# dscripka/openWakeWord

Hardware: NVIDIA H100
Metric: 80ms audio-frames/sec (concurrent streams) (higher is better)
Workload: dtype f16 operands / f32 accumulate (mel, BN, LayerNorm, sigmoid in f32; heads' first layer as fp16 hi/lo split = f32-grade)

## Files before the change

### openwakeword_b200/csrc/cnn_tc_inc.cu

```cuda
#include "oww_internal.h"
#include "tc_common.cuh"
#include "mel_device.cuh"
#include <cmath>
#include <cstring>
#include <type_traits>

namespace {

constexpr int kIncEpiWarps = 16;
constexpr int kIncThreads = kIncEpiWarps * 32;
constexpr int kIncMaxG = 7;
constexpr int kMelNF = 2;

__device__ __forceinline__ __half2 u32_as_half2(uint32_t v) {
    return __halves2half2(__ushort_as_half((unsigned short)(v & 0xFFFFu)), __ushort_as_half((unsigned short)(v >> 16)));
}

struct IncArgs {
    IncPlan plan;
    const float* mel; const int* mel_count; int64_t mel_stride; int mel_mask; int back;
    const float* w0; const float* s0; const float* b0;
    const uint8_t* wblob;
    const uint4* tails_in; uint4* tails_out;
    float* emb;
    int B;
    const int* live_chunks; int live_min;
    long long* dbg_clock;
// ... 73 lines not shown
        mbar_expect_tx(hfull(slot), bytes);
        bulk_g2s(smem_u32(smem + a.hring_off + slot * a.hslot_bytes), src, bytes, hfull(slot));
        ++hchunk_p;
        return true;
    };

    const int et = threadIdx.x;
    uint32_t epar[2] = {0, 0};
    uint32_t epi_tails_par = 0, mma_tails_par = 0;
    uint32_t hf_par = 0; int hchunk_e = 0;
    for (int grp = blockIdx.x; grp < P.n_groups; grp += gridDim.x) {
        const uint4* tin = a.tails_in + (int64_t)grp * P.tail_units;
        uint4* tout = a.tails_out + (int64_t)grp * P.tail_units;
        int* s_cnt = reinterpret_cast<int*>(smem + 512);
        int* s_live = s_cnt + 16;
        float* s_mel = reinterpret_cast<float*>(smem + P.scratch_off + 6144);
        if (a.dbg_clock && blockIdx.x == 0 && grp == 0 && et == 0) a.dbg_clock[101] = clock64();
        named_bar_sync(2, kIncEpiWarps * 32);
        if (et < G) {
            const int b = grp * G + et;
            s_live[et] = b < a.B && (!a.live_chunks || a.live_chunks[b] >= a.live_min);
        }
        named_bar_sync(2, kIncEpiWarps * 32);
        if (fused) {
            uint8_t* sc = smem + P.scratch_off;
            float2* s_tw = reinterpret_cast<float2*>(sc);
            float* s_win = reinterpret_cast<float*>(sc + 4096);
            uint8_t* s_work = smem + 2048 + warp * (kMelNF * kMelFrameScratch);
            float* s_floor = s_mel + G * 256;
            int seen_v = 1;
            for (int i = et; i < 512; i += kIncEpiWarps * 32) { s_tw[i] = a.mel_twiddle[i]; s_win[i] = a.mel_window[i]; }
            if (et < G) {
                const int b = grp * G + et;
                s_cnt[et] = s_live[et] ? a.mel_count_rw[b] : 0;
                s_cnt[8 + et] = s_live[et] ? a.feat_count[b] : 0;
                seen_v = s_live[et] ? a.seen[b] : 1;
                s_live[8 + et] = s_live[et] && seen_v == 0;
            }
            named_bar_sync(2, kIncEpiWarps * 32);
            const int my_start = a.mel_start[lane], my_len = a.mel_len[lane];
            const float* my_w = a.mel_w + lane * OWW_MEL_MAXSUPPORT;
            for (int fi = warp * kMelNF; fi < G * 8; fi += kIncEpiWarps * kMelNF) {
                const int16_t* tl[kMelNF]; const int16_t* bd[kMelNF]; int fr[kMelNF]; float db[kMelNF];
#pragma unroll
                for (int i = 0; i < kMelNF; ++i) {
                    const int fj = fi + i < G * 8 ? fi + i : fi;
                    int b = grp * G + (fj >> 3);
                    if (b >= a.B) b = grp * G;
                    tl[i] = a.tail + (int64_t)b * OWW_TAIL; bd[i] = a.pcm + (int64_t)b * a.pcm_stride; fr[i] = fj & 7;
                }
                long long* st = (a.dbg_clock && blockIdx.x == 0 && grp == 0 && warp == 0 && fi == 0) ? a.dbg_clock + 92 : nullptr;
                mel_frames_db<kMelNF>(tl, OWW_TAIL, bd, fr, s_work, s_tw, s_win, a.mel_kmax, my_start, my_len, my_w, lane, db, st);
#pragma unroll
                for (int i = 0; i < kMelNF; ++i)
                    if (fi + i < G * 8) s_mel[(fi + i) * 32 + lane] = db[i];
            }
            named_bar_sync(2, kIncEpiWarps * 32);
            if (a.dbg_clock && blockIdx.x == 0 && grp == 0 && et == 0) a.dbg_clock[97] = clock64();
            constexpr int kTW = OWW_TAIL / 2;
            const bool al = ((size_t)a.pcm & 3) == 0 && (a.pcm_stride & 1) == 0;
            uint32_t tv[4]; int ti[4];
#pragma unroll
            for (int u = 0; u < 4; ++u) {
                const int i = et + u * kIncEpiWarps * 32;
                ti[u] = -1; tv[u] = 0;
                if (i < G * kTW) {
                    const int g = i / kTW, k = i - g * kTW, b = grp * G + g;
// ... 644 lines not shown
    for (int l = 1; l < NL; ++l) {
        const int above = wsz(l + 1) > wsz(l - 1) ? wsz(l + 1) : wsz(l - 1);
        P.L[l].w_smem = (l & 1) ? kTop - wsz(l) : kTop - above - wsz(l);
    }
    for (int l = 1; l < NL; ++l) {
        int w_low = P.L[l].w_smem;
        if (l + 1 < NL && P.L[l + 1].w_smem < w_low) w_low = P.L[l + 1].w_smem;
        if (act_high[l] > w_low || act_high[l - 1] > P.L[l].w_smem)
            return oww_fail(ctx, OWW_EUNSUPPORTED, "fused-CNN smem plan does not fit at layer %d (G=%d)", l, G);
        if (l >= 2 && wsz(l) < wsz(l - 1)) return oww_fail(ctx, OWW_EUNSUPPORTED, "weight sizes must not shrink with depth");
    }
    if (NL == OWW_N_CONV) {
        int off = kActBase + r8(size_nx[0]) * 16;
        const int work_end = kActBase + kIncEpiWarps * kMelNF * kMelFrameScratch;
        if (work_end > off) off = (work_end + 127) & ~127;
        const int need_b = 6144 + G * 256 * 4 + 64;
        P.scratch_off = (off + need_b <= P.L[1].w_smem && off + need_b <= P.L[2].w_smem) ? off : 0;
    }
    P.w_total_bytes = (int)w_off;
    P.smem_bytes = kTop;
    *out = P;
    return OWW_OK;
}

int oww_inc_setup(oww_ctx* ctx, const float* h_blob) {
    IncPlan P;
    int rc = oww_inc_build_plan(ctx, 1, 1, OWW_N_CONV, &P);
    if (rc) return rc;
    std::vector<uint8_t> blob(P.w_total_bytes, 0);
    size_t off = 0;
    for (int li = 0; li < OWW_N_CONV; ++li) {
// ... 249 lines not shown
```

### openwakeword_b200/csrc/mel.cu

```cuda
#include "oww_internal.h"
#include "tc_common.cuh"
#include "mel_device.cuh"
#include <climits>
#include <cmath>
#include <cstring>

namespace {

constexpr int kWarps = 8;
constexpr int kThreads = kWarps * 32;

struct MelDev {
    const float* window;
    const float2* twiddle;
    const int* mel_start;
    const int* mel_len;
    const float* mel_w;
    int kmax;
};

__global__ void __launch_bounds__(kThreads, 5) mel_kernel(MelLaunch p, MelDev c) {
    __shared__ __align__(16) uint8_t s_work[kWarps][kMelFrameScratch];
    __shared__ float2 s_tw[512];
    __shared__ float s_win[512];
    __shared__ float s_red[kWarps];

    pdl_trigger();
    const int clip = p.ids ? p.ids[blockIdx.x] : blockIdx.x;
    const int tid = threadIdx.x, lane = tid & 31, warp = tid >> 5;
    if (p.live && p.live[clip] < p.live_min) {
        pdl_wait();
        return;
    }

    for (int i = tid; i < 512; i += kThreads) { s_tw[i] = c.twiddle[i]; s_win[i] = c.window[i]; }

    const bool streaming = p.tail != nullptr;
    const int prefix = streaming ? OWW_TAIL : 0;
    const int seen0 = streaming ? p.seen[clip] : 0;
    const bool fresh = streaming && seen0 == 0;
    const int total = prefix + p.n_body;
    const int T = (total - OWW_FFT_N) / OWW_HOP + 1;
    const int f0 = fresh ? 3 : 0;
    const int nrows = T - f0;
    const bool one_pass = nrows <= kWarps;
    const int16_t* body = p.body + (int64_t)clip * p.body_stride;
    const int16_t* tail = streaming ? p.tail + (int64_t)clip * OWW_TAIL : nullptr;
    const int row0 = p.out_count ? p.out_count[clip] : 0;
    float* out = p.out + (int64_t)clip * p.out_stride;
    __syncthreads();

    const int my_start = c.mel_start[lane];
    const int my_len = c.mel_len[lane];
    const float* my_w = c.mel_w + lane * OWW_MEL_MAXSUPPORT;
    float vmax = -INFINITY, kept = 0.f;

    for (int f = f0 + warp; f < T; f += kWarps) {
        float db;
        mel_frames_db<1>(&tail, prefix, &body, &f, s_work[warp], s_tw, s_win, c.kmax, my_start, my_len, my_w, lane, &db);
        vmax = fmaxf(vmax, db);
        if (one_pass) { kept = db; continue; }
        pdl_wait();
        const int r = f - f0;
        const int slot = p.out_rows_mask >= 0 ? ((row0 + r) & p.out_rows_mask) : r;
        out[(int64_t)slot * OWW_MEL_BINS + lane] = db;
    }
#pragma unroll
    for (int o = 16; o > 0; o >>= 1) vmax = fmaxf(vmax, __shfl_xor_sync(0xffffffffu, vmax, o));
    if (lane == 0) s_red[warp] = vmax;
    __syncthreads();
    float m = s_red[0];
#pragma unroll
    for (int w = 1; w < kWarps; ++w) m = fmaxf(m, s_red[w]);
    const float floor_db = m - 80.0f;
    int16_t tv[(OWW_TAIL + kThreads - 1) / kThreads];
#pragma unroll
    for (int u = 0; u < (OWW_TAIL + kThreads - 1) / kThreads; ++u) {
        const int i = tid + u * kThreads;
        tv[u] = streaming && i < OWW_TAIL ? __ldg(body + (p.n_body - OWW_TAIL + i)) : (int16_t)0;
    }
    pdl_wait();
    if (one_pass) {
        if (warp < nrows) {
            float v = fmaxf(kept, floor_db);
            if (p.affine) v = v / 10.0f + 2.0f;
            const int slot = p.out_rows_mask >= 0 ? ((row0 + warp) & p.out_rows_mask) : warp;
            out[(int64_t)slot * OWW_MEL_BINS + lane] = v;
        }
    } else {
        for (int i = tid; i < nrows * OWW_MEL_BINS; i += kThreads) {
            const int r = i >> 5, col = i & 31;
            const int slot = p.out_rows_mask >= 0 ? ((row0 + r) & p.out_rows_mask) : r;
            float* q = out + (int64_t)slot * OWW_MEL_BINS + col;
            float v = fmaxf(__ldcg(q), floor_db);
            if (p.affine) v = v / 10.0f + 2.0f;
            *q = v;
        }
    }
    if (streaming) {
        int16_t* tw = p.tail + (int64_t)clip * OWW_TAIL;
#pragma unroll
        for (int u = 0; u < (OWW_TAIL + kThreads - 1) / kThreads; ++u)
            if (tid + u * kThreads < OWW_TAIL) tw[tid + u * kThreads] = tv[u];
        if (tid == 0) {
            p.out_count[clip] = oww_wrap_count(row0 + nrows);
            const int sn = seen0 + p.n_chunks;
            p.seen[clip] = sn > (1 << 30) ? (1 << 30) : sn;
        }
    }
}

__host__ __device__ __forceinline__ int clip_frame_step(int f) { return f < 5 ? 0 : (f - 5) / 8 + 1; }
__host__ __device__ __forceinline__ int clip_group(int f, int chunk) {
    return (int)oww_call_first_step(oww_call_of_step(clip_frame_step(f), chunk), chunk);
}
__host__ __device__ __forceinline__ int clip_first_group(int k0, int chunk) { return clip_group(8 * k0 > 71 ? 8 * k0 - 71 : 0, chunk); }

__global__ void __launch_bounds__(kThreads) mel_clip_kernel(const int16_t* pcm, const int64_t* clip_off, const int* clip_len, int pad,
                                                            int chunk, int k0, int k1, float* out, int64_t out_stride, MelDev c) {
    extern __shared__ __align__(16) uint8_t dyn[];
    float2 (*s_buf)[2][256] = reinterpret_cast<float2 (*)[2][256]>(dyn);
    float2* s_tw = reinterpret_cast<float2*>(dyn + kWarps * 2 * 256 * sizeof(float2));
    float* s_win = reinterpret_cast<float*>(s_tw + 512);
    float (*s_pow)[264] = reinterpret_cast<float (*)[264]>(s_win + 512);
    int16_t (*s_frame)[512] = reinterpret_cast<int16_t (*)[512]>(s_pow + kWarps);
    int* s_gmax = reinterpret_cast<int*>(s_frame + kWarps);
    const int clip = blockIdx.x;
    const int tid = threadIdx.x, lane = tid & 31, warp = tid >> 5;
    const int v0 = 8 * k0;
    const int g0 = clip_first_group(k0, chunk);
    const int f0 = g0 == 0 ? 0 : 8 * g0 - 3;
    const int n_frames = 8 * k1 - 3;
    for (int i = tid; i < 512; i += kThreads) { s_tw[i] = c.twiddle[i]; s_win[i] = c.window[i]; }
    for (int i = tid; i < k1 - g0; i += kThreads) s_gmax[i] = INT_MIN;
    const int16_t* body = pcm + clip_off[clip];
    const int n_samples = clip_len[clip];
    float* o = out + (int64_t)clip * out_stride;
    for (int i = tid; i < (71 - v0) * 32; i += kThreads) o[i] = 1.0f;
    __syncthreads();
    const int my_start = c.mel_start[lane];
    const int my_len = c.mel_len[lane];
    const float* my_w = c.mel_w + lane * OWW_MEL_MAXSUPPORT;
    auto enc = [](float v) { int i = __float_as_int(v); return i >= 0 ? i : i ^ 0x7FFFFFFF; };
    for (int f = f0 + warp; f < n_frames; f += kWarps) {
        for (int j = lane; j < 512; j += 32) {
            const int64_t p = (int64_t)f * OWW_HOP + j - pad;
            s_frame[warp][j] = (p >= 0 && p < n_samples) ? body[p] : (int16_t)0;
        }
        __syncwarp();
        const float db = mel_frame_db<false>(nullptr, 0, s_frame[warp], 0, s_buf[warp][0], s_buf[warp][1], s_pow[warp], s_tw, s_win, c.kmax,
                                      my_start, my_len, my_w, lane);
        if (71 + f >= v0) o[(int64_t)(71 + f - v0) * 32 + lane] = db;
        float m = db;
#pragma unroll
        for (int k = 16; k > 0; k >>= 1) m = fmaxf(m, __shfl_xor_sync(0xffffffffu, m, k));
        if (lane == 0) atomicMax(&s_gmax[clip_group(f, chunk) - g0], enc(m));
        __syncwarp();
    }
    __syncthreads();
    const int fw = max(f0, v0 - 71);
    for (int i = tid; i < (n_frames - fw) * 32; i += kThreads) {
        const int f = fw + (i >> 5);
        const int e = s_gmax[clip_group(f, chunk) - g0];
        const float gmax = __int_as_float(e >= 0 ? e : e ^ 0x7FFFFFFF);
        float* q = o + (int64_t)(71 + f - v0) * 32 + (i & 31);
        *q = fmaxf(*q, gmax - 80.0f) / 10.0f + 2.0f;
    }
}

double hz_to_mel(double f) {
    const double f_sp = 200.0 / 3.0, min_log_hz = 1000.0, min_log_mel = min_log_hz / f_sp;
    const double logstep = std::log(6.4) / 27.0;
    return f >= min_log_hz ? min_log_mel + std::log(f / min_log_hz) / logstep : f / f_sp;
}
double mel_to_hz(double m) {
    const double f_sp = 200.0 / 3.0, min_log_hz = 1000.0, min_log_mel = min_log_hz / f_sp;
    const double logstep = std::log(6.4) / 27.0;
    return m >= min_log_mel ? min_log_hz * std::exp(logstep * (m - min_log_mel)) : f_sp * m;
}

}

int oww_mel_launch(oww_ctx* ctx, const MelLaunch& p, cudaStream_t s) {
    if (!ctx->mel_loaded) return oww_fail(ctx, OWW_EINVAL, "mel constants not loaded");
    const int prefix = p.tail ? OWW_TAIL : 0;
    if (prefix + p.n_body < OWW_FFT_N) return oww_fail(ctx, OWW_EINVAL, "clip shorter than 512 samples");
    if (p.n_clips <= 0) return OWW_OK;
    MelDev c{ctx->d_window, ctx->d_twiddle, ctx->d_mel_start, ctx->d_mel_len, ctx->d_mel_w, ctx->mel_kmax};
    OWW_CUDA(ctx, oww_launch_pdl(p.pdl, mel_kernel, dim3(p.n_clips), dim3(kThreads), 0, s, p, c));
    OWW_LAUNCH_CHECK(ctx);
    return OWW_OK;
}

int oww_mel_clips_launch(oww_ctx* ctx, const int16_t* d_pcm, const int64_t* d_off, const int* d_len, int n_clips, int pad,
                         int chunk, int k0, int k1, float* d_out, int64_t out_stride, cudaStream_t s) {
    if (!ctx->mel_loaded) return oww_fail(ctx, OWW_EINVAL, "mel constants not loaded");
    if (n_clips <= 0 || k1 <= k0) return OWW_OK;
    if (k0 < 0 || k1 - k0 > 8192 || chunk < 1 || oww_call_first_step(oww_call_of_step(k1, chunk), chunk) != k1)
        return oww_fail(ctx, OWW_EINVAL, "step range [%d,%d) is not a bulk frontend segment", k0, k1);
    MelDev c{ctx->d_window, ctx->d_twiddle, ctx->d_mel_start, ctx->d_mel_len, ctx->d_mel_w, ctx->mel_kmax};
    const size_t smem = (size_t)kWarps * 2 * 256 * sizeof(float2) + 512 * sizeof(float2) + 512 * sizeof(float) +
                        (size_t)kWarps * 264 * sizeof(float) + (size_t)kWarps * 512 * sizeof(int16_t) +
                        (size_t)(k1 - clip_first_group(k0, chunk)) * sizeof(int);
    if (!ctx->mel_clip_attr_set) {
        OWW_CUDA(ctx, cudaFuncSetAttribute(mel_clip_kernel, cudaFuncAttributeMaxDynamicSharedMemorySize, 100 * 1024));
        ctx->mel_clip_attr_set = true;
    }
    mel_clip_kernel<<<n_clips, kThreads, smem, s>>>(d_pcm, d_off, d_len, pad, chunk, k0, k1, d_out, out_stride, c);
    OWW_LAUNCH_CHECK(ctx);
    return OWW_OK;
}

extern "C" int oww_load_mel(oww_ctx* ctx, const float* h_window512, const float* h_mel_fb) {
    if (!ctx) return OWW_EINVAL;
    OWW_CUDA(ctx, cudaSetDevice(ctx->device));
    const double kPi = 3.14159265358979323846;
    std::vector<float> win(512, 0.f);
    if (h_window512) {
        std::memcpy(win.data(), h_window512, 512 * sizeof(float));
    } else {
        for (int n = 0; n < 400; ++n) win[56 + n] = (float)(0.5 - 0.5 * std::cos(2.0 * kPi * n / 400.0));
    }
    std::vector<float2> tw(512);
// ... 54 lines not shown
```

### openwakeword_b200/csrc/mel_device.cuh

```cuda
#pragma once
#include <cuda_runtime.h>
#include <cstdint>
#include "oww_internal.h"

namespace {

__device__ __forceinline__ float2 cmul(float2 a, float2 b) {
    return make_float2(__fmaf_rn(a.x, b.x, -__fmul_rn(a.y, b.y)), __fmaf_rn(a.x, b.y, __fmul_rn(a.y, b.x)));
}

template <bool kBodyGlobal = true>
__device__ __forceinline__ float mel_frame_db(const int16_t* tail, int prefix, const int16_t* body, int f, float2* a, float2* b,
                                              float* pw_buf, const float2* s_tw, const float* s_win, int kmax, int my_start,
                                              int my_len, const float* my_w, int lane) {
#pragma unroll
        for (int j = 0; j < 8; ++j) {
            const int n = lane + 32 * j;
            const int s0 = f * OWW_HOP + 2 * n;
            float x0, x1;
            if (s0 + 1 < prefix) { x0 = (float)tail[s0]; x1 = (float)tail[s0 + 1]; }
            else if (s0 >= prefix) {
                if (kBodyGlobal) { x0 = (float)__ldg(body + (s0 - prefix)); x1 = (float)__ldg(body + (s0 + 1 - prefix)); }
                else { x0 = (float)body[s0 - prefix]; x1 = (float)body[s0 + 1 - prefix]; }
            }
            else { x0 = (float)tail[s0]; x1 = kBodyGlobal ? (float)__ldg(body) : (float)body[0]; }
            a[n] = make_float2(__fmul_rn(x0, s_win[2 * n]), __fmul_rn(x1, s_win[2 * n + 1]));
        }
        __syncwarp();
#pragma unroll
        for (int Ns = 1; Ns < 256; Ns *= 4) {
            const int tstep = 128 / Ns;
#pragma unroll
            for (int jj = 0; jj < 2; ++jj) {
                const int j = lane + 32 * jj;
                const int k = j & (Ns - 1);
                float2 v0 = a[j];
                float2 v1 = cmul(a[j + 64], s_tw[k * tstep]);
                float2 v2 = cmul(a[j + 128], s_tw[2 * k * tstep]);
                float2 v3 = cmul(a[j + 192], s_tw[3 * k * tstep]);
                float2 a0 = make_float2(v0.x + v2.x, v0.y + v2.y);
                float2 a1 = make_float2(v0.x - v2.x, v0.y - v2.y);
                float2 a2 = make_float2(v1.x + v3.x, v1.y + v3.y);
                float2 d = make_float2(v1.x - v3.x, v1.y - v3.y);
                float2 a3 = make_float2(d.y, -d.x);
                const int dst = (j / Ns) * Ns * 4 + k;
                b[dst] = make_float2(a0.x + a2.x, a0.y + a2.y);
                b[dst + Ns] = make_float2(a1.x + a3.x, a1.y + a3.y);
                b[dst + 2 * Ns] = make_float2(a0.x - a2.x, a0.y - a2.y);
                b[dst + 3 * Ns] = make_float2(a1.x - a3.x, a1.y - a3.y);
            }
            __syncwarp();
            float2* t = a; a = b; b = t;
        }
        for (int k = lane; k < kmax; k += 32) {
            float pw;
            if (k == 256) {
                const float x = a[0].x - a[0].y;
                pw = __fmul_rn(x, x);
            } else {
                const float2 zk = a[k & 255];
                const float2 zc = a[(256 - k) & 255];
                const float2 xe = make_float2(0.5f * (zk.x + zc.x), 0.5f * (zk.y - zc.y));
                const float2 dd = make_float2(zk.x - zc.x, zk.y + zc.y);
                const float2 xo = make_float2(0.5f * dd.y, -0.5f * dd.x);
                const float2 t2 = cmul(s_tw[k], xo);
                const float re = __fadd_rn(xe.x, t2.x), im = __fadd_rn(xe.y, t2.y);
                pw = __fmaf_rn(re, re, __fmul_rn(im, im));
            }
            pw_buf[k] = pw;
        }
        __syncwarp();
        float acc = 0.f;
        for (int i = 0; i < my_len; ++i) acc = fmaf(pw_buf[my_start + i], my_w[i], acc);
        const float db = 10.0f * logf(fmaxf(acc, 1e-10f)) / logf(10.0f);
    return db;
}

#ifndef OWW_FFT_SWZ
#define OWW_FFT_SWZ 1
#endif
__device__ __forceinline__ int fswz(int e) {
#if OWW_FFT_SWZ
    return e ^ (((e >> 4) & 3) * 5);
#else
    return e;
#endif
}

constexpr int kMelFrameScratch = 2048 + 2048;
template <int NF>
__device__ __forceinline__ void mel_frames_db(const int16_t* const* tail, int prefix, const int16_t* const* body, const int* f,
                                              uint8_t* bufs, const float2* s_tw, const float* s_win, int kmax, int my_start,
                                              int my_len, const float* my_w, int lane, float* db, long long* stamps = nullptr) {
    float2* a[NF]; float2* b[NF]; float* pw[NF];
    if (stamps && lane == 0) stamps[0] = clock64();
#pragma unroll
    for (int i = 0; i < NF; ++i) {
        a[i] = reinterpret_cast<float2*>(bufs + i * kMelFrameScratch);
        b[i] = a[i] + 256;
        pw[i] = reinterpret_cast<float*>(b[i]);
    }
    bool al[NF];
#pragma unroll
    for (int i = 0; i < NF; ++i) al[i] = (((size_t)body[i] | (size_t)tail[i]) & 3) == 0 && (prefix & 1) == 0;
    uint32_t raw[8][NF];
#pragma unroll
    for (int j = 0; j < 8; ++j) {
        const int n = lane + 32 * j;
#pragma unroll
        for (int i = 0; i < NF; ++i) {
            const int s0 = f[i] * OWW_HOP + 2 * n;
            if (al[i]) {
                raw[j][i] = s0 + 1 < prefix ? *reinterpret_cast<const uint32_t*>(tail[i] + s0)
                                            : __ldg(reinterpret_cast<const uint32_t*>(body[i] + (s0 - prefix)));
            } else {
                unsigned short u0, u1;
                if (s0 + 1 < prefix) { u0 = (unsigned short)tail[i][s0]; u1 = (unsigned short)tail[i][s0 + 1]; }
                else if (s0 >= prefix) { u0 = (unsigned short)__ldg(body[i] + (s0 - prefix)); u1 = (unsigned short)__ldg(body[i] + (s0 + 1 - prefix)); }
                else { u0 = (unsigned short)tail[i][s0]; u1 = (unsigned short)__ldg(body[i]); }
                raw[j][i] = (uint32_t)u0 | ((uint32_t)u1 << 16);
            }
        }
    }
#pragma unroll
    for (int j = 0; j < 8; ++j) {
        const int n = lane + 32 * j;
        const float2 wn = *reinterpret_cast<const float2*>(s_win + 2 * n);
#pragma unroll
        for (int i = 0; i < NF; ++i) {
            const float x0 = (float)(short)(raw[j][i] & 0xFFFFu), x1 = (float)(short)(raw[j][i] >> 16);
            a[i][fswz(n)] = make_float2(__fmul_rn(x0, wn.x), __fmul_rn(x1, wn.y));
        }
    }
    __syncwarp();
    if (stamps && lane == 0) stamps[1] = clock64();
#pragma unroll
    for (int Ns = 1; Ns < 256; Ns *= 4) {
        const int tstep = 128 / Ns;
        float2 t1 = make_float2(1.f, 0.f), t2 = t1, t3 = t1;
        if (Ns > 1 && Ns <= 32) { const int k = lane & (Ns - 1); t1 = s_tw[k * tstep]; t2 = s_tw[2 * k * tstep]; t3 = s_tw[3 * k * tstep]; }
#pragma unroll
        for (int jj = 0; jj < 2; ++jj) {
            const int j = lane + 32 * jj;
            const int k = j & (Ns - 1);
            if (Ns > 32) { t1 = s_tw[k * tstep]; t2 = s_tw[2 * k * tstep]; t3 = s_tw[3 * k * tstep]; }
            const int dst = (j / Ns) * Ns * 4 + k;
            const int sj = fswz(j);
            const int d0 = fswz(dst), d1 = fswz(dst + Ns), d2 = fswz(dst + 2 * Ns), d3 = fswz(dst + 3 * Ns);
#pragma unroll
            for (int i = 0; i < NF; ++i) {
                const float2 v0 = a[i][sj];
                float2 v1 = a[i][sj + 64], v2 = a[i][sj + 128], v3 = a[i][sj + 192];
                if (Ns > 1) { v1 = cmul(v1, t1); v2 = cmul(v2, t2); v3 = cmul(v3, t3); }
                float2 a0 = make_float2(v0.x + v2.x, v0.y + v2.y);
                float2 a1 = make_float2(v0.x - v2.x, v0.y - v2.y);
                float2 a2 = make_float2(v1.x + v3.x, v1.y + v3.y);
                float2 d = make_float2(v1.x - v3.x, v1.y - v3.y);
                float2 a3 = make_float2(d.y, -d.x);
                b[i][d0] = make_float2(a0.x + a2.x, a0.y + a2.y);
                b[i][d1] = make_float2(a1.x + a3.x, a1.y + a3.y);
                b[i][d2] = make_float2(a0.x - a2.x, a0.y - a2.y);
                b[i][d3] = make_float2(a1.x - a3.x, a1.y - a3.y);
            }
        }
        __syncwarp();
#pragma unroll
        for (int i = 0; i < NF; ++i) { float2* t = a[i]; a[i] = b[i]; b[i] = t; }
    }
    if (stamps && lane == 0) stamps[2] = clock64();
    for (int k = lane; k < kmax; k += 32) {
#pragma unroll
        for (int i = 0; i < NF; ++i) {
            float p;
            if (k == 256) {
                const float x = a[i][fswz(0)].x - a[i][fswz(0)].y;
                p = __fmul_rn(x, x);
            } else {
                const float2 zk = a[i][fswz(k & 255)];
                const float2 zc = a[i][fswz((256 - k) & 255)];
                const float2 xe = make_float2(0.5f * (zk.x + zc.x), 0.5f * (zk.y - zc.y));
                const float2 dd = make_float2(zk.x - zc.x, zk.y + zc.y);
                const float2 xo = make_float2(0.5f * dd.y, -0.5f * dd.x);
                const float2 t2 = cmul(s_tw[k], xo);
                const float re = __fadd_rn(xe.x, t2.x), im = __fadd_rn(xe.y, t2.y);
                p = __fmaf_rn(re, re, __fmul_rn(im, im));
            }
            pw[i][k] = p;
        }
    }
    __syncwarp();
    if (stamps && lane == 0) stamps[3] = clock64();
    float acc[NF];
#pragma unroll
    for (int i = 0; i < NF; ++i) acc[i] = 0.f;
    for (int q = 0; q < my_len; q += 4) {
        const float4 w4 = __ldg(reinterpret_cast<const float4*>(my_w + q));
        const float w[4] = {w4.x, w4.y, w4.z, w4.w};
#pragma unroll
        for (int e = 0; e < 4; ++e)
            if (q + e < my_len) {
#pragma unroll
                for (int i = 0; i < NF; ++i) acc[i] = fmaf(pw[i][my_start + q + e], w[e], acc[i]);
            }
    }
#pragma unroll
    for (int i = 0; i < NF; ++i) db[i] = 10.0f * logf(fmaxf(acc[i], 1e-10f)) / logf(10.0f);
    __syncwarp();
    if (stamps && lane == 0) stamps[4] = clock64();
}

}
```

Measured before the change: 6.195 million.

## Rewrite mel FFT as register-resident warp-shuffle FFT, drop smem staging

Replaces the shared-memory radix-4 FFT in the mel frontend with a register-resident FFT that exchanges data across lanes via shuffles, keeping only a per-frame power spectrum in shared memory. Twiddles and window are read through __ldg instead of being staged in shared memory per block. The standalone mel kernel now packs two streams per CTA and processes two frames per warp, and the fused CNN path shrinks its mel scratch and drops to one frame per warp. This reduces shared-memory traffic, syncs and per-block setup, at the cost of higher register pressure and more shuffle instructions.

```diff
diff --git a/openwakeword_b200/csrc/cnn_tc_inc.cu b/openwakeword_b200/csrc/cnn_tc_inc.cu
--- a/openwakeword_b200/csrc/cnn_tc_inc.cu
+++ b/openwakeword_b200/csrc/cnn_tc_inc.cu
@@ -10,7 +10,7 @@
 constexpr int kIncEpiWarps = 16;
 constexpr int kIncThreads = kIncEpiWarps * 32;
 constexpr int kIncMaxG = 7;
-constexpr int kMelNF = 2;
+constexpr int kMelNF = 1;
 
 __device__ __forceinline__ __half2 u32_as_half2(uint32_t v) {
     return __halves2half2(__ushort_as_half((unsigned short)(v & 0xFFFFu)), __ushort_as_half((unsigned short)(v >> 16)));
@@ -114,7 +114,7 @@
         uint4* tout = a.tails_out + (int64_t)grp * P.tail_units;
         int* s_cnt = reinterpret_cast<int*>(smem + 512);
         int* s_live = s_cnt + 16;
-        float* s_mel = reinterpret_cast<float*>(smem + P.scratch_off + 6144);
+        float* s_mel = reinterpret_cast<float*>(smem + P.scratch_off);
         if (a.dbg_clock && blockIdx.x == 0 && grp == 0 && et == 0) a.dbg_clock[101] = clock64();
         named_bar_sync(2, kIncEpiWarps * 32);
         if (et < G) {
@@ -123,13 +123,9 @@
         }
         named_bar_sync(2, kIncEpiWarps * 32);
         if (fused) {
-            uint8_t* sc = smem + P.scratch_off;
-            float2* s_tw = reinterpret_cast<float2*>(sc);
-            float* s_win = reinterpret_cast<float*>(sc + 4096);
-            uint8_t* s_work = smem + 2048 + warp * (kMelNF * kMelFrameScratch);
+            float* s_pw = reinterpret_cast<float*>(smem + 2048 + warp * (kMelNF * kMelFrameScratch));
             float* s_floor = s_mel + G * 256;
             int seen_v = 1;
-            for (int i = et; i < 512; i += kIncEpiWarps * 32) { s_tw[i] = a.mel_twiddle[i]; s_win[i] = a.mel_window[i]; }
             if (et < G) {
                 const int b = grp * G + et;
                 s_cnt[et] = s_live[et] ? a.mel_count_rw[b] : 0;
@@ -150,7 +146,8 @@
                     tl[i] = a.tail + (int64_t)b * OWW_TAIL; bd[i] = a.pcm + (int64_t)b * a.pcm_stride; fr[i] = fj & 7;
                 }
                 long long* st = (a.dbg_clock && blockIdx.x == 0 && grp == 0 && warp == 0 && fi == 0) ? a.dbg_clock + 92 : nullptr;
-                mel_frames_db<kMelNF>(tl, OWW_TAIL, bd, fr, s_work, s_tw, s_win, a.mel_kmax, my_start, my_len, my_w, lane, db, st);
+                mel_frames_db<kMelNF>(TailBodyPairs<kMelNF>(tl, OWW_TAIL, bd, fr), a.mel_twiddle, a.mel_window, s_pw, a.mel_kmax,
+                                      my_start, my_len, my_w, lane, db, st);
 #pragma unroll
                 for (int i = 0; i < kMelNF; ++i)
                     if (fi + i < G * 8) s_mel[(fi + i) * 32 + lane] = db[i];
@@ -825,7 +822,7 @@
         int off = kActBase + r8(size_nx[0]) * 16;
         const int work_end = kActBase + kIncEpiWarps * kMelNF * kMelFrameScratch;
         if (work_end > off) off = (work_end + 127) & ~127;
-        const int need_b = 6144 + G * 256 * 4 + 64;
+        const int need_b = G * 256 * 4 + 64;
         P.scratch_off = (off + need_b <= P.L[1].w_smem && off + need_b <= P.L[2].w_smem) ? off : 0;
     }
     P.w_total_bytes = (int)w_off;
diff --git a/openwakeword_b200/csrc/mel.cu b/openwakeword_b200/csrc/mel.cu
--- a/openwakeword_b200/csrc/mel.cu
+++ b/openwakeword_b200/csrc/mel.cu
@@ -7,8 +7,13 @@
 
 namespace {
 
-constexpr int kWarps = 8;
+constexpr int kNF = 2;
+constexpr int kStreamWarps = 4;
+constexpr int kStreamsPerCta = 2;
+constexpr int kWarps = kStreamWarps * kStreamsPerCta;
 constexpr int kThreads = kWarps * 32;
+constexpr int kStreamThreads = kStreamWarps * 32;
+constexpr int kPassRows = kStreamWarps * kNF;
 
 struct MelDev {
     const float* window;
@@ -19,76 +24,85 @@
     int kmax;
 };
 
-__global__ void __launch_bounds__(kThreads, 5) mel_kernel(MelLaunch p, MelDev c) {
-    __shared__ __align__(16) uint8_t s_work[kWarps][kMelFrameScratch];
-    __shared__ float2 s_tw[512];
-    __shared__ float s_win[512];
-    __shared__ float s_red[kWarps];
+__global__ void __launch_bounds__(kThreads, 3) mel_kernel(MelLaunch p, MelDev c) {
+    __shared__ __align__(16) float s_pw[kWarps][kNF * kMelFrameScratch / 4];
+    __shared__ float s_red[kStreamsPerCta][kStreamWarps];
 
     pdl_trigger();
-    const int clip = p.ids ? p.ids[blockIdx.x] : blockIdx.x;
-    const int tid = threadIdx.x, lane = tid & 31, warp = tid >> 5;
-    if (p.live && p.live[clip] < p.live_min) {
-        pdl_wait();
-        return;
-    }
-
-    for (int i = tid; i < 512; i += kThreads) { s_tw[i] = c.twiddle[i]; s_win[i] = c.window[i]; }
+    const int tid = threadIdx.x, lane = tid & 31;
+    const int warp = __shfl_sync(0xffffffffu, tid >> 5, 0);
+    const int sg = warp / kStreamWarps, sw = warp % kStreamWarps, st = tid % kStreamThreads;
+    const int j = blockIdx.x * kStreamsPerCta + sg;
+    const int clip = j < p.n_clips ? (p.ids ? p.ids[j] : j) : 0;
+    const bool dead = __shfl_sync(0xffffffffu, j >= p.n_clips || (p.live && p.live[clip] < p.live_min), 0);
 
     const bool streaming = p.tail != nullptr;
     const int prefix = streaming ? OWW_TAIL : 0;
-    const int seen0 = streaming ? p.seen[clip] : 0;
+    const int seen0 = __shfl_sync(0xffffffffu, streaming && !dead ? p.seen[clip] : 0, 0);
     const bool fresh = streaming && seen0 == 0;
     const int total = prefix + p.n_body;
     const int T = (total - OWW_FFT_N) / OWW_HOP + 1;
     const int f0 = fresh ? 3 : 0;
     const int nrows = T - f0;
-    const bool one_pass = nrows <= kWarps;
+    const bool one_pass = nrows <= kPassRows;
     const int16_t* body = p.body + (int64_t)clip * p.body_stride;
     const int16_t* tail = streaming ? p.tail + (int64_t)clip * OWW_TAIL : nullptr;
-    const int row0 = p.out_count ? p.out_count[clip] : 0;
+    const int row0_early = p.out_count && !dead && !one_pass ? p.out_count[clip] : 0;
     float* out = p.out + (int64_t)clip * p.out_stride;
-    __syncthreads();
 
     const int my_start = c.mel_start[lane];
     const int my_len = c.mel_len[lane];
     const float* my_w = c.mel_w + lane * OWW_MEL_MAXSUPPORT;
-    float vmax = -INFINITY, kept = 0.f;
-
-    for (int f = f0 + warp; f < T; f += kWarps) {
-        float db;
-        mel_frames_db<1>(&tail, prefix, &body, &f, s_work[warp], s_tw, s_win, c.kmax, my_start, my_len, my_w, lane, &db);
-        vmax = fmaxf(vmax, db);
-        if (one_pass) { kept = db; continue; }
-        pdl_wait();
-        const int r = f - f0;
-        const int slot = p.out_rows_mask >= 0 ? ((row0 + r) & p.out_rows_mask) : r;
-        out[(int64_t)slot * OWW_MEL_BINS + lane] = db;
-    }
+    float vmax = -INFINITY, kept[kNF];
+
+    for (int fb = f0 + sw * kNF; !dead && fb < T; fb += kPassRows) {
+        const int16_t* tl[kNF]; const int16_t* bd[kNF]; int fr[kNF]; float db[kNF];
+#pragma unroll
+        for (int i = 0; i < kNF; ++i) { tl[i] = tail; bd[i] = body; fr[i] = fb + i < T ? fb + i : fb; }
+        mel_frames_db<kNF>(TailBodyPairs<kNF>(tl, prefix, bd, fr), c.twiddle, c.window, s_pw[warp], c.kmax, my_start, my_len,
+                           my_w, lane, db);
+#pragma unroll
+        for (int i = 0; i < kNF; ++i) {
+            if (fb + i >= T) break;
+            vmax = fmaxf(vmax, db[i]);
+            kept[i] = db[i];
+            if (one_pass) continue;
+            pdl_wait();
+            const int r = fb + i - f0;
+            const int slot = p.out_rows_mask >= 0 ? ((row0_early + r) & p.out_rows_mask) : r;
+            out[(int64_t)slot * OWW_MEL_BINS + lane] = db[i];
+        }
+    }
+    const int row0 = one_pass ? (p.out_count && !dead ? p.out_count[clip] : 0) : row0_early;
 #pragma unroll
     for (int o = 16; o > 0; o >>= 1) vmax = fmaxf(vmax, __shfl_xor_sync(0xffffffffu, vmax, o));
-    if (lane == 0) s_red[warp] = vmax;
+    if (lane == 0) s_red[sg][sw] = vmax;
     __syncthreads();
-    float m = s_red[0];
-#pragma unroll
-    for (int w = 1; w < kWarps; ++w) m = fmaxf(m, s_red[w]);
+    float m = s_red[sg][0];
+#pragma unroll
+    for (int w = 1; w < kStreamWarps; ++w) m = fmaxf(m, s_red[sg][w]);
     const float floor_db = m - 80.0f;
-    int16_t tv[(OWW_TAIL + kThreads - 1) / kThreads];
-#pragma unroll
-    for (int u = 0; u < (OWW_TAIL + kThreads - 1) / kThreads; ++u) {
-        const int i = tid + u * kThreads;
-        tv[u] = streaming && i < OWW_TAIL ? __ldg(body + (p.n_body - OWW_TAIL + i)) : (int16_t)0;
+    constexpr int kTailPer = (OWW_TAIL + kStreamThreads - 1) / kStreamThreads;
+    int16_t tv[kTailPer];
+#pragma unroll
+    for (int u = 0; u < kTailPer; ++u) {
+        const int i = st + u * kStreamThreads;
+        tv[u] = streaming && !dead && i < OWW_TAIL ? __ldg(body + (p.n_body - OWW_TAIL + i)) : (int16_t)0;
     }
     pdl_wait();
+    if (dead) return;
     if (one_pass) {
-        if (warp < nrows) {
-            float v = fmaxf(kept, floor_db);
+#pragma unroll
+        for (int i = 0; i < kNF; ++i) {
+            const int r = sw * kNF + i;
+            if (r >= nrows) break;
+            float v = fmaxf(kept[i], floor_db);
             if (p.affine) v = v / 10.0f + 2.0f;
-            const int slot = p.out_rows_mask >= 0 ? ((row0 + warp) & p.out_rows_mask) : warp;
+            const int slot = p.out_rows_mask >= 0 ? ((row0 + r) & p.out_rows_mask) : r;
             out[(int64_t)slot * OWW_MEL_BINS + lane] = v;
         }
     } else {
-        for (int i = tid; i < nrows * OWW_MEL_BINS; i += kThreads) {
+        for (int i = st; i < nrows * OWW_MEL_BINS; i += kStreamThreads) {
             const int r = i >> 5, col = i & 31;
             const int slot = p.out_rows_mask >= 0 ? ((row0 + r) & p.out_rows_mask) : r;
             float* q = out + (int64_t)slot * OWW_MEL_BINS + col;
@@ -100,9 +114,9 @@
     if (streaming) {
         int16_t* tw = p.tail + (int64_t)clip * OWW_TAIL;
 #pragma unroll
-        for (int u = 0; u < (OWW_TAIL + kThreads - 1) / kThreads; ++u)
-            if (tid + u * kThreads < OWW_TAIL) tw[tid + u * kThreads] = tv[u];
-        if (tid == 0) {
+        for (int u = 0; u < kTailPer; ++u)
+            if (st + u * kStreamThreads < OWW_TAIL) tw[st + u * kStreamThreads] = tv[u];
+        if (st == 0) {
             p.out_count[clip] = oww_wrap_count(row0 + nrows);
             const int sn = seen0 + p.n_chunks;
             p.seen[clip] = sn > (1 << 30) ? (1 << 30) : sn;
@@ -116,50 +130,62 @@
 }
 __host__ __device__ __forceinline__ int clip_first_group(int k0, int chunk) { return clip_group(8 * k0 > 71 ? 8 * k0 - 71 : 0, chunk); }
 
-__global__ void __launch_bounds__(kThreads) mel_clip_kernel(const int16_t* pcm, const int64_t* clip_off, const int* clip_len, int pad,
-                                                            int chunk, int k0, int k1, float* out, int64_t out_stride, MelDev c) {
+constexpr int kClipWarps = 8;
+constexpr int kClipThreads = kClipWarps * 32;
+
+template <int NF>
+struct PaddedClipPairs {
+    const int16_t* body; int n; int64_t s[NF];
+    __device__ __forceinline__ uint32_t operator()(int i, int k) const {
+        const int64_t q = s[i] + 2 * k;
+        const unsigned short u0 = q >= 0 && q < n ? (unsigned short)__ldg(body + q) : 0;
+        const unsigned short u1 = q + 1 >= 0 && q + 1 < n ? (unsigned short)__ldg(body + q + 1) : 0;
+        return (uint32_t)u0 | ((uint32_t)u1 << 16);
+    }
+};
+
+__global__ void __launch_bounds__(kClipThreads) mel_clip_kernel(const int16_t* pcm, const int64_t* clip_off, const int* clip_len, int pad,
+                                                                int chunk, int k0, int k1, float* out, int64_t out_stride, MelDev c) {
     extern __shared__ __align__(16) uint8_t dyn[];
-    float2 (*s_buf)[2][256] = reinterpret_cast<float2 (*)[2][256]>(dyn);
-    float2* s_tw = reinterpret_cast<float2*>(dyn + kWarps * 2 * 256 * sizeof(float2));
-    float* s_win = reinterpret_cast<float*>(s_tw + 512);
-    float (*s_pow)[264] = reinterpret_cast<float (*)[264]>(s_win + 512);
-    int16_t (*s_frame)[512] = reinterpret_cast<int16_t (*)[512]>(s_pow + kWarps);
-    int* s_gmax = reinterpret_cast<int*>(s_frame + kWarps);
+    float (*s_pw)[kNF * kMelFrameScratch / 4] = reinterpret_cast<float (*)[kNF * kMelFrameScratch / 4]>(dyn);
+    int* s_gmax = reinterpret_cast<int*>(s_pw + kClipWarps);
     const int clip = blockIdx.x;
-    const int tid = threadIdx.x, lane = tid & 31, warp = tid >> 5;
+    const int tid = threadIdx.x, lane = tid & 31;
+    const int warp = __shfl_sync(0xffffffffu, tid >> 5, 0);
     const int v0 = 8 * k0;
     const int g0 = clip_first_group(k0, chunk);
     const int f0 = g0 == 0 ? 0 : 8 * g0 - 3;
     const int n_frames = 8 * k1 - 3;
-    for (int i = tid; i < 512; i += kThreads) { s_tw[i] = c.twiddle[i]; s_win[i] = c.window[i]; }
-    for (int i = tid; i < k1 - g0; i += kThreads) s_gmax[i] = INT_MIN;
+    for (int i = tid; i < k1 - g0; i += kClipThreads) s_gmax[i] = INT_MIN;
     const int16_t* body = pcm + clip_off[clip];
     const int n_samples = clip_len[clip];
     float* o = out + (int64_t)clip * out_stride;
-    for (int i = tid; i < (71 - v0) * 32; i += kThreads) o[i] = 1.0f;
+    for (int i = tid; i < (71 - v0) * 32; i += kClipThreads) o[i] = 1.0f;
     __syncthreads();
     const int my_start = c.mel_start[lane];
     const int my_len = c.mel_len[lane];
     const float* my_w = c.mel_w + lane * OWW_MEL_MAXSUPPORT;
     auto enc = [](float v) { int i = __float_as_int(v); return i >= 0 ? i : i ^ 0x7FFFFFFF; };
-    for (int f = f0 + warp; f < n_frames; f += kWarps) {
-        for (int j = lane; j < 512; j += 32) {
-            const int64_t p = (int64_t)f * OWW_HOP + j - pad;
-            s_frame[warp][j] = (p >= 0 && p < n_samples) ? body[p] : (int16_t)0;
-        }
-        __syncwarp();
-        const float db = mel_frame_db<false>(nullptr, 0, s_frame[warp], 0, s_buf[warp][0], s_buf[warp][1], s_pow[warp], s_tw, s_win, c.kmax,
-                                      my_start, my_len, my_w, lane);
-        if (71 + f >= v0) o[(int64_t)(71 + f - v0) * 32 + lane] = db;
-        float m = db;
-#pragma unroll
-        for (int k = 16; k > 0; k >>= 1) m = fmaxf(m, __shfl_xor_sync(0xffffffffu, m, k));
-        if (lane == 0) atomicMax(&s_gmax[clip_group(f, chunk) - g0], enc(m));
-        __syncwarp();
+    for (int fb = f0 + warp * kNF; fb < n_frames; fb += kClipWarps * kNF) {
+        PaddedClipPairs<kNF> pairs{body, n_samples, {}};
+#pragma unroll
+        for (int i = 0; i < kNF; ++i) pairs.s[i] = (int64_t)(fb + i < n_frames ? fb + i : fb) * OWW_HOP - pad;
+        float db[kNF];
+        mel_frames_db<kNF>(pairs, c.twiddle, c.window, s_pw[warp], c.kmax, my_start, my_len, my_w, lane, db);
+#pragma unroll
+        for (int i = 0; i < kNF; ++i) {
+            const int f = fb + i;
+            if (f >= n_frames) break;
+            if (71 + f >= v0) o[(int64_t)(71 + f - v0) * 32 + lane] = db[i];
+            float m = db[i];
+#pragma unroll
+            for (int k = 16; k > 0; k >>= 1) m = fmaxf(m, __shfl_xor_sync(0xffffffffu, m, k));
+            if (lane == 0) atomicMax(&s_gmax[clip_group(f, chunk) - g0], enc(m));
+        }
     }
     __syncthreads();
     const int fw = max(f0, v0 - 71);
-    for (int i = tid; i < (n_frames - fw) * 32; i += kThreads) {
+    for (int i = tid; i < (n_frames - fw) * 32; i += kClipThreads) {
         const int f = fw + (i >> 5);
         const int e = s_gmax[clip_group(f, chunk) - g0];
         const float gmax = __int_as_float(e >= 0 ? e : e ^ 0x7FFFFFFF);
@@ -187,7 +213,7 @@
     if (prefix + p.n_body < OWW_FFT_N) return oww_fail(ctx, OWW_EINVAL, "clip shorter than 512 samples");
     if (p.n_clips <= 0) return OWW_OK;
     MelDev c{ctx->d_window, ctx->d_twiddle, ctx->d_mel_start, ctx->d_mel_len, ctx->d_mel_w, ctx->mel_kmax};
-    OWW_CUDA(ctx, oww_launch_pdl(p.pdl, mel_kernel, dim3(p.n_clips), dim3(kThreads), 0, s, p, c));
+    OWW_CUDA(ctx, oww_launch_pdl(p.pdl, mel_kernel, dim3((p.n_clips + kStreamsPerCta - 1) / kStreamsPerCta), dim3(kThreads), 0, s, p, c));
     OWW_LAUNCH_CHECK(ctx);
     return OWW_OK;
 }
@@ -199,14 +225,12 @@
     if (k0 < 0 || k1 - k0 > 8192 || chunk < 1 || oww_call_first_step(oww_call_of_step(k1, chunk), chunk) != k1)
         return oww_fail(ctx, OWW_EINVAL, "step range [%d,%d) is not a bulk frontend segment", k0, k1);
     MelDev c{ctx->d_window, ctx->d_twiddle, ctx->d_mel_start, ctx->d_mel_len, ctx->d_mel_w, ctx->mel_kmax};
-    const size_t smem = (size_t)kWarps * 2 * 256 * sizeof(float2) + 512 * sizeof(float2) + 512 * sizeof(float) +
-                        (size_t)kWarps * 264 * sizeof(float) + (size_t)kWarps * 512 * sizeof(int16_t) +
-                        (size_t)(k1 - clip_first_group(k0, chunk)) * sizeof(int);
+    const size_t smem = (size_t)kClipWarps * kNF * kMelFrameScratch + (size_t)(k1 - clip_first_group(k0, chunk)) * sizeof(int);
     if (!ctx->mel_clip_attr_set) {
         OWW_CUDA(ctx, cudaFuncSetAttribute(mel_clip_kernel, cudaFuncAttributeMaxDynamicSharedMemorySize, 100 * 1024));
         ctx->mel_clip_attr_set = true;
     }
-    mel_clip_kernel<<<n_clips, kThreads, smem, s>>>(d_pcm, d_off, d_len, pad, chunk, k0, k1, d_out, out_stride, c);
+    mel_clip_kernel<<<n_clips, kClipThreads, smem, s>>>(d_pcm, d_off, d_len, pad, chunk, k0, k1, d_out, out_stride, c);
     OWW_LAUNCH_CHECK(ctx);
     return OWW_OK;
 }
diff --git a/openwakeword_b200/csrc/mel_device.cuh b/openwakeword_b200/csrc/mel_device.cuh
--- a/openwakeword_b200/csrc/mel_device.cuh
+++ b/openwakeword_b200/csrc/mel_device.cuh
@@ -9,183 +9,142 @@
     return make_float2(__fmaf_rn(a.x, b.x, -__fmul_rn(a.y, b.y)), __fmaf_rn(a.x, b.y, __fmul_rn(a.y, b.x)));
 }
 
-template <bool kBodyGlobal = true>
-__device__ __forceinline__ float mel_frame_db(const int16_t* tail, int prefix, const int16_t* body, int f, float2* a, float2* b,
-                                              float* pw_buf, const float2* s_tw, const float* s_win, int kmax, int my_start,
-                                              int my_len, const float* my_w, int lane) {
+__device__ __forceinline__ int mel_fft_lo(int lane) {
+    return ((lane >> 4) & 1) | (lane & 2) | ((lane >> 1) & 4) | ((lane << 1) & 8) | ((lane & 1) << 4);
+}
+__host__ __device__ constexpr int mel_fft_hi(int r) { return ((r >> 1) & 1) | ((r & 1) << 1) | (r & 4); }
+
+template <int B, int C, int NF>
+__device__ __forceinline__ void fft_xchg(float2 (&v)[NF][8], int lane) {
+    const bool up = (lane >> B) & 1;
 #pragma unroll
-        for (int j = 0; j < 8; ++j) {
-            const int n = lane + 32 * j;
-            const int s0 = f * OWW_HOP + 2 * n;
-            float x0, x1;
-            if (s0 + 1 < prefix) { x0 = (float)tail[s0]; x1 = (float)tail[s0 + 1]; }
-            else if (s0 >= prefix) {
-                if (kBodyGlobal) { x0 = (float)__ldg(body + (s0 - prefix)); x1 = (float)__ldg(body + (s0 + 1 - prefix)); }
-                else { x0 = (float)body[s0 - prefix]; x1 = (float)body[s0 + 1 - prefix]; }
-            }
-            else { x0 = (float)tail[s0]; x1 = kBodyGlobal ? (float)__ldg(body) : (float)body[0]; }
-            a[n] = make_float2(__fmul_rn(x0, s_win[2 * n]), __fmul_rn(x1, s_win[2 * n + 1]));
+    for (int r = 0; r < 8; ++r) {
+        constexpr int c = 1 << C;
+        if (r & c) continue;
+#pragma unroll
+        for (int i = 0; i < NF; ++i) {
+            const float2 s = up ? v[i][r] : v[i][r | c];
+            const float2 g = make_float2(__shfl_xor_sync(0xffffffffu, s.x, 1 << B), __shfl_xor_sync(0xffffffffu, s.y, 1 << B));
+            if (up) v[i][r] = g; else v[i][r | c] = g;
         }
-        __syncwarp();
-#pragma unroll
-        for (int Ns = 1; Ns < 256; Ns *= 4) {
-            const int tstep = 128 / Ns;
-#pragma unroll
-            for (int jj = 0; jj < 2; ++jj) {
-                const int j = lane + 32 * jj;
-                const int k = j & (Ns - 1);
-                float2 v0 = a[j];
-                float2 v1 = cmul(a[j + 64], s_tw[k * tstep]);
-                float2 v2 = cmul(a[j + 128], s_tw[2 * k * tstep]);
-                float2 v3 = cmul(a[j + 192], s_tw[3 * k * tstep]);
-                float2 a0 = make_float2(v0.x + v2.x, v0.y + v2.y);
-                float2 a1 = make_float2(v0.x - v2.x, v0.y - v2.y);
-                float2 a2 = make_float2(v1.x + v3.x, v1.y + v3.y);
-                float2 d = make_float2(v1.x - v3.x, v1.y - v3.y);
-                float2 a3 = make_float2(d.y, -d.x);
-                const int dst = (j / Ns) * Ns * 4 + k;
-                b[dst] = make_float2(a0.x + a2.x, a0.y + a2.y);
-                b[dst + Ns] = make_float2(a1.x + a3.x, a1.y + a3.y);
-                b[dst + 2 * Ns] = make_float2(a0.x - a2.x, a0.y - a2.y);
-                b[dst + 3 * Ns] = make_float2(a1.x - a3.x, a1.y - a3.y);
-            }
-            __syncwarp();
-            float2* t = a; a = b; b = t;
-        }
-        for (int k = lane; k < kmax; k += 32) {
-            float pw;
-            if (k == 256) {
-                const float x = a[0].x - a[0].y;
-                pw = __fmul_rn(x, x);
-            } else {
-                const float2 zk = a[k & 255];
-                const float2 zc = a[(256 - k) & 255];
-                const float2 xe = make_float2(0.5f * (zk.x + zc.x), 0.5f * (zk.y - zc.y));
-                const float2 dd = make_float2(zk.x - zc.x, zk.y + zc.y);
-                const float2 xo = make_float2(0.5f * dd.y, -0.5f * dd.x);
-                const float2 t2 = cmul(s_tw[k], xo);
-                const float re = __fadd_rn(xe.x, t2.x), im = __fadd_rn(xe.y, t2.y);
-                pw = __fmaf_rn(re, re, __fmul_rn(im, im));
-            }
-            pw_buf[k] = pw;
-        }
-        __syncwarp();
-        float acc = 0.f;
-        for (int i = 0; i < my_len; ++i) acc = fmaf(pw_buf[my_start + i], my_w[i], acc);
-        const float db = 10.0f * logf(fmaxf(acc, 1e-10f)) / logf(10.0f);
-    return db;
+    }
 }
 
-#ifndef OWW_FFT_SWZ
-#define OWW_FFT_SWZ 1
-#endif
-__device__ __forceinline__ int fswz(int e) {
-#if OWW_FFT_SWZ
-    return e ^ (((e >> 4) & 3) * 5);
-#else
-    return e;
-#endif
+template <bool kTw, int D6, int D7, int DJ, int NF>
+__device__ __forceinline__ void fft_pass(float2 (&v)[NF][8], const float2 (&t)[2][3]) {
+#pragma unroll
+    for (int jj = 0; jj < 2; ++jj) {
+        constexpr int m6 = 1 << D6, m7 = 1 << D7;
+        const int r0 = jj << DJ;
+#pragma unroll
+        for (int i = 0; i < NF; ++i) {
+            const float2 v0 = v[i][r0];
+            float2 v1 = v[i][r0 | m6], v2 = v[i][r0 | m7], v3 = v[i][r0 | m6 | m7];
+            if (kTw) { v1 = cmul(v1, t[jj][0]); v2 = cmul(v2, t[jj][1]); v3 = cmul(v3, t[jj][2]); }
+            const float2 a0 = make_float2(v0.x + v2.x, v0.y + v2.y);
+            const float2 a1 = make_float2(v0.x - v2.x, v0.y - v2.y);
+            const float2 a2 = make_float2(v1.x + v3.x, v1.y + v3.y);
+            const float2 d = make_float2(v1.x - v3.x, v1.y - v3.y);
+            const float2 a3 = make_float2(d.y, -d.x);
+            v[i][r0] = make_float2(a0.x + a2.x, a0.y + a2.y);
+            v[i][r0 | m6] = make_float2(a1.x + a3.x, a1.y + a3.y);
+            v[i][r0 | m7] = make_float2(a0.x - a2.x, a0.y - a2.y);
+            v[i][r0 | m6 | m7] = make_float2(a1.x - a3.x, a1.y - a3.y);
+        }
+    }
 }
 
-constexpr int kMelFrameScratch = 2048 + 2048;
+__device__ __forceinline__ void fft_twiddles(const float2* tw, int k0, int k1, int tstep, float2 (&t)[2][3]) {
+#pragma unroll
+    for (int m = 1; m <= 3; ++m) { t[0][m - 1] = __ldg(tw + m * k0 * tstep); t[1][m - 1] = __ldg(tw + m * k1 * tstep); }
+}
+
 template <int NF>
-__device__ __forceinline__ void mel_frames_db(const int16_t* const* tail, int prefix, const int16_t* const* body, const int* f,
-                                              uint8_t* bufs, const float2* s_tw, const float* s_win, int kmax, int my_start,
-                                              int my_len, const float* my_w, int lane, float* db, long long* stamps = nullptr) {
-    float2* a[NF]; float2* b[NF]; float* pw[NF];
+struct TailBodyPairs {
+    const int16_t* tail[NF]; const int16_t* body[NF]; int s[NF]; bool al[NF]; int prefix;
+    __device__ __forceinline__ TailBodyPairs(const int16_t* const* tl, int pre, const int16_t* const* bd, const int* f) : prefix(pre) {
+#pragma unroll
+        for (int i = 0; i < NF; ++i) {
+            tail[i] = tl[i]; body[i] = bd[i]; s[i] = f[i] * OWW_HOP;
+            al[i] = (((size_t)bd[i] | (size_t)tl[i]) & 3) == 0 && (pre & 1) == 0;
+        }
+    }
+    __device__ __forceinline__ uint32_t operator()(int i, int n) const {
+        const int s0 = s[i] + 2 * n;
+        if (al[i])
+            return s0 + 1 < prefix ? *reinterpret_cast<const uint32_t*>(tail[i] + s0)
+                                   : __ldg(reinterpret_cast<const uint32_t*>(body[i] + (s0 - prefix)));
+        unsigned short u0, u1;
+        if (s0 + 1 < prefix) { u0 = (unsigned short)tail[i][s0]; u1 = (unsigned short)tail[i][s0 + 1]; }
+        else if (s0 >= prefix) { u0 = (unsigned short)__ldg(body[i] + (s0 - prefix)); u1 = (unsigned short)__ldg(body[i] + (s0 + 1 - prefix)); }
+        else { u0 = (unsigned short)tail[i][s0]; u1 = (unsigned short)__ldg(body[i]); }
+        return (uint32_t)u0 | ((uint32_t)u1 << 16);
+    }
+};
+
+constexpr int kMelFrameScratch = 256 * sizeof(float);
+template <int NF, class Pairs>
+__device__ __forceinline__ void mel_frames_db(const Pairs& pair, const float2* tw, const float* win, float* pw, int kmax,
+                                              int my_start, int my_len, const float* my_w, int lane, float* db,
+                                              long long* stamps = nullptr) {
     if (stamps && lane == 0) stamps[0] = clock64();
-#pragma unroll
-    for (int i = 0; i < NF; ++i) {
-        a[i] = reinterpret_cast<float2*>(bufs + i * kMelFrameScratch);
-        b[i] = a[i] + 256;
-        pw[i] = reinterpret_cast<float*>(b[i]);
-    }
-    bool al[NF];
-#pragma unroll
-    for (int i = 0; i < NF; ++i) al[i] = (((size_t)body[i] | (size_t)tail[i]) & 3) == 0 && (prefix & 1) == 0;
     uint32_t raw[8][NF];
 #pragma unroll
-    for (int j = 0; j < 8; ++j) {
-        const int n = lane + 32 * j;
+    for (int r = 0; r < 8; ++r)
+#pragma unroll
+        for (int i = 0; i < NF; ++i) raw[r][i] = pair(i, lane + 32 * r);
+    float2 v[NF][8];
+#pragma unroll
+    for (int r = 0; r < 8; ++r) {
+        const float2 wn = __ldg(reinterpret_cast<const float2*>(win) + lane + 32 * r);
 #pragma unroll
         for (int i = 0; i < NF; ++i) {
-            const int s0 = f[i] * OWW_HOP + 2 * n;
-            if (al[i]) {
-                raw[j][i] = s0 + 1 < prefix ? *reinterpret_cast<const uint32_t*>(tail[i] + s0)
-                                            : __ldg(reinterpret_cast<const uint32_t*>(body[i] + (s0 - prefix)));
-            } else {
-                unsigned short u0, u1;
-                if (s0 + 1 < prefix) { u0 = (unsigned short)tail[i][s0]; u1 = (unsigned short)tail[i][s0 + 1]; }
-                else if (s0 >= prefix) { u0 = (unsigned short)__ldg(body[i] + (s0 - prefix)); u1 = (unsigned short)__ldg(body[i] + (s0 + 1 - prefix)); }
-                else { u0 = (unsigned short)tail[i][s0]; u1 = (unsigned short)__ldg(body[i]); }
-                raw[j][i] = (uint32_t)u0 | ((uint32_t)u1 << 16);
-            }
+            const float x0 = (float)(short)(raw[r][i] & 0xFFFFu), x1 = (float)(short)(raw[r][i] >> 16);
+            v[i][r] = make_float2(__fmul_rn(x0, wn.x), __fmul_rn(x1, wn.y));
         }
     }
+    if (stamps && lane == 0) stamps[1] = clock64();
+    const int l0 = (lane >> 4) & 1, l2 = (lane >> 3) & 1, l3 = (lane >> 2) & 1;
+    float2 t[2][3];
+    fft_pass<false, 1, 2, 0>(v, t);
+    fft_xchg<4, 1>(v, lane);
+    fft_twiddles(tw, l0, l0 | 2, 32, t);
+    fft_pass<true, 1, 0, 2>(v, t);
+    fft_xchg<2, 0>(v, lane);
+    fft_xchg<3, 1>(v, lane);
+    fft_twiddles(tw, l0 | (l2 << 2) | (l3 << 3), l0 | 2 | (l2 << 2) | (l3 << 3), 8, t);
+    fft_pass<true, 0, 1, 2>(v, t);
+    fft_xchg<0, 0>(v, lane);
+    fft_xchg<1, 2>(v, lane);
+    const int k3 = mel_fft_lo(lane);
+    fft_twiddles(tw, k3, k3 | 32, 2, t);
+    fft_pass<true, 0, 2, 1>(v, t);
+    if (stamps && lane == 0) stamps[2] = clock64();
+    const int lo = k3, src = mel_fft_lo((32 - lo) & 31);
+    float p256[NF] = {};
 #pragma unroll
-    for (int j = 0; j < 8; ++j) {
-        const int n = lane + 32 * j;
-        const float2 wn = *reinterpret_cast<const float2*>(s_win + 2 * n);
+    for (int h = 0; h < 8; ++h) {
+        if (32 * h >= kmax) break;
+        const int r = mel_fft_hi(h), rc = mel_fft_hi((8 - h) & 7), k = lo + 32 * h;
+        const float2 twk = __ldg(tw + k);
 #pragma unroll
         for (int i = 0; i < NF; ++i) {
-            const float x0 = (float)(short)(raw[j][i] & 0xFFFFu), x1 = (float)(short)(raw[j][i] >> 16);
-            a[i][fswz(n)] = make_float2(__fmul_rn(x0, wn.x), __fmul_rn(x1, wn.y));
+            const float2 zk = v[i][r];
+            float2 zc = make_float2(__shfl_sync(0xffffffffu, v[i][r ^ 7].x, src), __shfl_sync(0xffffffffu, v[i][r ^ 7].y, src));
+            if (lo == 0) zc = v[i][rc];
+            const float2 xe = make_float2(0.5f * (zk.x + zc.x), 0.5f * (zk.y - zc.y));
+            const float2 dd = make_float2(zk.x - zc.x, zk.y + zc.y);
+            const float2 xo = make_float2(0.5f * dd.y, -0.5f * dd.x);
+            const float2 t2 = cmul(twk, xo);
+            const float re = __fadd_rn(xe.x, t2.x), im = __fadd_rn(xe.y, t2.y);
+            if (k < kmax) pw[i * 256 + k] = __fmaf_rn(re, re, __fmul_rn(im, im));
         }
     }
-    __syncwarp();
-    if (stamps && lane == 0) stamps[1] = clock64();
-#pragma unroll
-    for (int Ns = 1; Ns < 256; Ns *= 4) {
-        const int tstep = 128 / Ns;
-        float2 t1 = make_float2(1.f, 0.f), t2 = t1, t3 = t1;
-        if (Ns > 1 && Ns <= 32) { const int k = lane & (Ns - 1); t1 = s_tw[k * tstep]; t2 = s_tw[2 * k * tstep]; t3 = s_tw[3 * k * tstep]; }
-#pragma unroll
-        for (int jj = 0; jj < 2; ++jj) {
-            const int j = lane + 32 * jj;
-            const int k = j & (Ns - 1);
-            if (Ns > 32) { t1 = s_tw[k * tstep]; t2 = s_tw[2 * k * tstep]; t3 = s_tw[3 * k * tstep]; }
-            const int dst = (j / Ns) * Ns * 4 + k;
-            const int sj = fswz(j);
-            const int d0 = fswz(dst), d1 = fswz(dst + Ns), d2 = fswz(dst + 2 * Ns), d3 = fswz(dst + 3 * Ns);
-#pragma unroll
-            for (int i = 0; i < NF; ++i) {
-                const float2 v0 = a[i][sj];
-                float2 v1 = a[i][sj + 64], v2 = a[i][sj + 128], v3 = a[i][sj + 192];
-                if (Ns > 1) { v1 = cmul(v1, t1); v2 = cmul(v2, t2); v3 = cmul(v3, t3); }
-                float2 a0 = make_float2(v0.x + v2.x, v0.y + v2.y);
-                float2 a1 = make_float2(v0.x - v2.x, v0.y - v2.y);
-                float2 a2 = make_float2(v1.x + v3.x, v1.y + v3.y);
-                float2 d = make_float2(v1.x - v3.x, v1.y - v3.y);
-                float2 a3 = make_float2(d.y, -d.x);
-                b[i][d0] = make_float2(a0.x + a2.x, a0.y + a2.y);
-                b[i][d1] = make_float2(a1.x + a3.x, a1.y + a3.y);
-                b[i][d2] = make_float2(a0.x - a2.x, a0.y - a2.y);
-                b[i][d3] = make_float2(a1.x - a3.x, a1.y - a3.y);
-            }
-        }
-        __syncwarp();
-#pragma unroll
-        for (int i = 0; i < NF; ++i) { float2* t = a[i]; a[i] = b[i]; b[i] = t; }
-    }
-    if (stamps && lane == 0) stamps[2] = clock64();
-    for (int k = lane; k < kmax; k += 32) {
+    if (kmax > 256) {
 #pragma unroll
         for (int i = 0; i < NF; ++i) {
-            float p;
-            if (k == 256) {
-                const float x = a[i][fswz(0)].x - a[i][fswz(0)].y;
-                p = __fmul_rn(x, x);
-            } else {
-                const float2 zk = a[i][fswz(k & 255)];
-                const float2 zc = a[i][fswz((256 - k) & 255)];
-                const float2 xe = make_float2(0.5f * (zk.x + zc.x), 0.5f * (zk.y - zc.y));
-                const float2 dd = make_float2(zk.x - zc.x, zk.y + zc.y);
-                const float2 xo = make_float2(0.5f * dd.y, -0.5f * dd.x);
-                const float2 t2 = cmul(s_tw[k], xo);
-                const float re = __fadd_rn(xe.x, t2.x), im = __fadd_rn(xe.y, t2.y);
-                p = __fmaf_rn(re, re, __fmul_rn(im, im));
-            }
-            pw[i][k] = p;
+            const float x = v[i][0].x - v[i][0].y;
+            p256[i] = __shfl_sync(0xffffffffu, __fmul_rn(x, x), 0);
         }
     }
     __syncwarp();
@@ -193,15 +152,22 @@
     float acc[NF];
 #pragma unroll
     for (int i = 0; i < NF; ++i) acc[i] = 0.f;
-    for (int q = 0; q < my_len; q += 4) {
+    const bool nyq = my_start + my_len > 256;
+    const int n_buf = nyq ? my_len - 1 : my_len;
+    for (int q = 0; q < n_buf; q += 4) {
         const float4 w4 = __ldg(reinterpret_cast<const float4*>(my_w + q));
         const float w[4] = {w4.x, w4.y, w4.z, w4.w};
 #pragma unroll
         for (int e = 0; e < 4; ++e)
-            if (q + e < my_len) {
+            if (q + e < n_buf) {
 #pragma unroll
-                for (int i = 0; i < NF; ++i) acc[i] = fmaf(pw[i][my_start + q + e], w[e], acc[i]);
+                for (int i = 0; i < NF; ++i) acc[i] = fmaf(pw[i * 256 + my_start + q + e], w[e], acc[i]);
             }
+    }
+    if (nyq) {
+        const float wl = __ldg(my_w + my_len - 1);
+#pragma unroll
+        for (int i = 0; i < NF; ++i) acc[i] = fmaf(p256[i], wl, acc[i]);
     }
 #pragma unroll
     for (int i = 0; i < NF; ++i) db[i] = 10.0f * logf(fmaxf(acc[i], 1e-10f)) / logf(10.0f);
```

After: 6.412 million, median of 6. 1.03x the previous value.
